# sdatkinson/NeuralAmpModelerCore

Measured on AMD Instinct MI355X. Metric: real-time audio streams (xRT) at 48 kHz, wavenet_a1_standard, higher is better.
Workload: dtype f32

## Files before the change

neuralampmodelercore_amd/csrc/aq_table.h:

```cpp
#pragma once

namespace namhip
{
namespace aq
{
constexpr int kC0 = 16, kC1 = 8;
constexpr int kBlockF = 64;
constexpr int kLayers = 10;
constexpr int kJobT = 10, kJobM0 = 11, kJobHead = 21, kJobs = 22;
constexpr int kRings = 20;
constexpr int kTable = 64;
constexpr int kNst = 16;
constexpr int kFirst[kNst + 1] = {0, 1, 2, 3, 4, 5, 6, 7, 8, 9, 10, 12, 14, 16, 18, 20, 22};
#ifdef NAM_AQ_SOW
constexpr int kStageOfWave[kNst] = {NAM_AQ_SOW};
#else
constexpr int kStageOfWave[kNst] = {0, 3, 6, 8, 1, 4, 7, 9, 2, 5, 11, 13, 15, 10, 12, 14};
#endif
static_assert(kFirst[kNst] == kJobs, "aq stage table");

constexpr bool is_big(int job) { return job < kLayers; }
constexpr bool is_small(int job) { return job >= kJobM0 && job < kJobHead; }
constexpr bool has_ring(int job) { return is_big(job) || is_small(job); }
constexpr int ring_id(int job) { return is_big(job) ? job : job - kJobM0 + kLayers; }
constexpr int dil(int job) { return has_ring(job) ? 1 << (is_big(job) ? job : job - kJobM0) : 0; }
constexpr int chans(int job) { return job <= kJobT ? kC0 : kC1; }
constexpr int ring_len(int job) { return 2 * dil(job) + kBlockF; }
constexpr int ring_off(int job)
{
  int o = kTable;
  for (int r = 0; r < ring_id(job); r++)
    o += (r < kLayers ? kC0 : kC1) * (2 * (1 << (r % kLayers)) + kBlockF);
  return o;
}
constexpr bool res(int job) { return is_big(job) ? dil(job) <= 64 : is_small(job) ? dil(job) <= 128 : false; }
constexpr int stage_of(int job)
{
  int s = 0;
  for (int k = 1; k < kNst; k++)
    if (job >= kFirst[k])
      s = k;
  return s;
}
constexpr bool starts_stage(int job) { return kFirst[stage_of(job)] == job; }
constexpr bool takes_area(int job) { return job > 0 && job < kJobHead && starts_stage(job) && !res(job); }
#if defined(NAM_AQ_DEPTH4_MASK)
constexpr int depth_in(int job) { return (is_big(job) && ((NAM_AQ_DEPTH4_MASK >> job) & 1)) ? 4 : 2; }
#elif defined(NAM_AQ_DEEP_Q)
constexpr int depth_in(int job) { return (is_big(job) && !res(job)) ? 4 : 2; }
#else
constexpr int depth_in(int) { return 2; }
#endif
constexpr int kMirror = 15;
constexpr int mirror_rows(int job) { return is_big(job) && res(job) ? kMirror : 0; }
constexpr int in_rows(int job) { return res(job) ? ring_len(job) + mirror_rows(job) : takes_area(job) ? (is_big(job) ? 16 * depth_in(job) : kBlockF) : 0; }
constexpr int plane_b(int job) { return (in_rows(job) * 16 + 255) / 256 * 256; }
constexpr int in_bytes(int job) { return plane_b(job) * (chans(job) / 4); }

constexpr int kTileT = 4 * 2 * 16;
constexpr int kTileM = 4 * 2 * 8;
constexpr int kWrOff = 0;
constexpr int kWhOff = kWrOff + kTileT;
constexpr int kMTiles = kWhOff + kTileT;
constexpr int kHeadTile = kMTiles + kLayers * 4 * kTileM;
constexpr int kMConsts = kHeadTile + kTileM;
constexpr int kTConsts = kMConsts + kLayers * 24;
constexpr int kBigConsts = kTConsts + 16;
constexpr int kBlockFloats = kBigConsts + kLayers * 64;
static_assert(kBlockFloats % 4 == 0, "aq weight block");

constexpr int kWB = 0;
constexpr int kFlagB = kWB + kBlockFloats * 4;
constexpr int kSlotB0 = kFlagB + 256;
constexpr int kSubSlot = 2 * 1024 + 128 + 16, kBigSlot = 4 * 1024 + 256 + 16, kSmallSlot = 2 * 1024 + 256 + 16;
constexpr int slot_bytes(int b) { return is_big(kFirst[b + 1]) ? (depth_in(kFirst[b + 1]) == 4 ? kBigSlot : kSubSlot) : kFirst[b + 1] == kJobT ? kBigSlot : kSmallSlot; }
constexpr int slot_b(int b)
{
  int o = kSlotB0;
  for (int i = 0; i < b; i++)
    o += slot_bytes(i);
  return o;
}
constexpr int kInB0 = (slot_b(kNst - 1) + 255) / 256 * 256;
constexpr int in_b(int job)
{
  int o = kInB0;
  for (int i = 0; i < job; i++)
    o += in_bytes(i);
  return o;
}
constexpr int kLdsBytes = in_b(kJobs);
static_assert(kLdsBytes <= 160 * 1024, "aq LDS layout");
constexpr bool mirrors_fit()
{
  for (int j = 0; j < kJobs; j++)
    if (mirror_rows(j) && ((ring_len(j) + kMirror) * 16 > plane_b(j) || ring_len(j) < 2 * 16 + kMirror))
      return false;
  return true;
}
static_assert(mirrors_fit(), "aq: a mirror lies behind its ring's live rows, inside the ring's plane");
static_assert(kFlagB % 16 == 0 && kSlotB0 % 16 == 0 && kSubSlot % 16 == 0 && kBigSlot % 16 == 0 && kSmallSlot % 16 == 0, "aq LDS alignment");
}
}
```

neuralampmodelercore_amd/csrc/kernel_a1_q.hip:

```cpp
#include "device_common.h"
#include "il_common.h"
#include "aq_table.h"

#ifndef NAM_AQ_SLEEP
#define NAM_AQ_SLEEP 1
#endif
#define NAM_AQ_STR2(x) #x
#define NAM_AQ_STR(x) NAM_AQ_STR2(x)

namespace namhip
{

constexpr float kAqT1 = 0.893229853513558f, kAqT2 = (float)(2.45550750702956 - 2.44506634652299 * 0.893229853513558);
#pragma clang fp contract(off)
template <int ACT_T>
__device__ __forceinline__ mf::f4 aq_act4(const mf::f4& v, float c_t1 = kAqT1, float c_t2 = kAqT2)
{
  mf::f4 r;
#pragma unroll
  for (int i = 0; i < 4; i++)
  {
    const float x = v[i];
    if constexpr (ACT_T == ACT_FASTTANH)
    {
      constexpr float kA1 = (float)(2.45550750702956 - 2.44506634652299 * 0.821226666969744);
      const float ax = __builtin_fabsf(x);
      const float q = __builtin_fmaf(ax, ax, 2.44506634652299f);
      const float w = __builtin_fmaf(0.814642734961073f, ax, 1.0f);
      const float t1 = __builtin_fmaf(0.821226666969744f, ax, c_t1);
      const float t2 = __builtin_fmaf(kA1, ax, c_t2);
      const float den = __builtin_fmaf(q, ax * w, 2.44506634652299f);
      const float n = __builtin_fmaf(t1, q, t2);
      r[i] = (n * __builtin_amdgcn_rcpf(den)) * x;
    }
    else
    {
      static_assert(ACT_T == ACT_TANH, "nam_a1_q_kernel is compiled for Fasttanh and Tanh");
      const float e = __builtin_amdgcn_exp2f(x * 2.885390081777927f);
      r[i] = __builtin_fmaf(-2.0f, __builtin_amdgcn_rcpf(e + 1.0f), 1.0f);
    }
  }
  return r;
}

#ifdef NAM_AQ_STEADY_PRIO
constexpr int kAqSteadyPrio[aq::kNst] = {NAM_AQ_STEADY_PRIO};
#else
constexpr int kAqSteadyPrio[aq::kNst] = {0, 0, 0, 0, 0, 0, 0, 0, 0, 0, 0, 0, 0, 0, 0, 0};
#endif
template <int SS>
__device__ __forceinline__ void aq_steady_prio()
{
  if constexpr (kAqSteadyPrio[SS] == 3)
    __builtin_amdgcn_s_setprio((short)3);
  else if constexpr (kAqSteadyPrio[SS] == 2)
    __builtin_amdgcn_s_setprio((short)2);
  else if constexpr (kAqSteadyPrio[SS] == 1)
    __builtin_amdgcn_s_setprio((short)1);
  else
    __builtin_amdgcn_s_setprio((short)0);
}

#ifndef NAM_AQ_STAG_SLEEP
#define NAM_AQ_STAG_SLEEP 24
#endif
template <int SS>
__device__ __forceinline__ void aq_stagger()
{
#ifdef NAM_AQ_STAG_FIXED
  if constexpr (SS > 0)
    __builtin_amdgcn_s_sleep(NAM_AQ_STAG_FIXED);
#endif
  if constexpr (SS > 0 && NAM_AQ_STAG_SLEEP > 0)
  {
#pragma unroll 1
    for (int r = 0; r < SS; r++)
      __builtin_amdgcn_s_sleep(NAM_AQ_STAG_SLEEP);
  }
}

namespace aq
{
constexpr int kNotReady = -(1 << 20);
constexpr int kNoRow = 1 << 26;
constexpr int kRowsMax = 1 << 20;
constexpr int far_jobs_before(int s, int job)
{
  int c = 0;
  for (int i = kFirst[s]; i < job; i++)
    c += (has_ring(i) && !res(i)) ? 1 : 0;
  return c;
}
constexpr int max_far_small()
{
  int m = 0;
  for (int s = 0; s < kNst; s++)
    if (is_small(kFirst[s]))
      m = far_jobs_before(s, kFirst[s + 1]) > m ? far_jobs_before(s, kFirst[s + 1]) : m;
  return m;
}
}

template <int ACT_T, bool WT, bool PERSIST, bool DBG = false, bool BANK = false>
__global__ __launch_bounds__(aq::kNst * 64) void nam_a1_q_kernel(const float* __restrict__ blob0, const A1Args a)
{
  long long dbg_t[8] = {0, 0, 0, 0, 0, 0, 0, 0};
  if constexpr (DBG)
    dbg_t[0] = clock64();
  using namespace mf;
  using il::kOob;
  using il::i4;
  constexpr int NST = aq::kNst;
  extern __shared__ __attribute__((aligned(16))) float lds_aq[];
  char* const lds = reinterpret_cast<char*>(lds_aq);
  const int tid = threadIdx.x;
  const int lane = tid & 63;
  const int wall = uni(tid >> 6);
  int S = 0;
#pragma unroll
  for (int i = 0; i < NST; i++)
    S = wall == i ? aq::kStageOfWave[i] : S;
  __builtin_amdgcn_s_setprio((short)0);
  if (wall >= 12)
    __builtin_amdgcn_s_setprio((short)3);
  else if (wall >= 8)
    __builtin_amdgcn_s_setprio((short)2);
  else if (wall >= 4)
    __builtin_amdgcn_s_setprio((short)1);
  const int stream = a.stream_map ? a.stream_map[blockIdx.x] : (int)blockIdx.x;
  const il::Weights wsrc = il::weights_of<BANK>(blob0, a, stream);
  const float* __restrict__ blob = wsrc.blob;
  float* st = a.state + (size_t)stream * a.state_stride;
  const int n_blocks = PERSIST ? (1 << 30) : (a.n_frames + kBlock - 1) / kBlock;

  const int frame = lane;
  const int g = lane >> 4, n = lane & 15;
  const unsigned g16 = (unsigned)g * 16u;
  const unsigned frame16 = (unsigned)frame * 16u;
  const unsigned cls64 = (unsigned)(lane & 3) * 64u;
  const unsigned cls128 = (unsigned)(lane & 3) * 128u;
  const float* in = a.in ? a.in + (size_t)stream * a.io_stride : nullptr;
  float* out = a.out ? a.out + (size_t)stream * a.io_stride : nullptr;
  const float head_scale = wsrc.head_scale;
  const int io_bytes = PERSIST ? 0x7ffffff0 : a.n_frames * 4;
  const auto rsrc_in = __builtin_amdgcn_make_buffer_rsrc((void*)(in ? in : st), 0, in ? io_bytes : 0, 0x00020000);
  const auto rsrc_out = __builtin_amdgcn_make_buffer_rsrc((void*)(out ? out : st), 0, out ? io_bytes : 0, 0x00020000);
  const unsigned long long in_addr = (unsigned long long)(in ? in : st);
  const i4 in_desc = {uni((int)(unsigned)in_addr), uni((int)(unsigned)(in_addr >> 32) & 0xffff), in ? io_bytes : 0, 0x00020000};
  int* wpos_tbl = reinterpret_cast<int*>(st);
  const int wposv = lane < aq::kRings ? wpos_tbl[lane] : 0;
  int* const flags = reinterpret_cast<int*>(lds + aq::kFlagB);

  constexpr int NT = 64;
  auto copy_block = [&](int first_float, int n_floats) {
    const f4* __restrict__ src = reinterpret_cast<const f4*>(blob + a.tiles_off + first_float);
    const int n4 = n_floats / 4;
    for (int i0 = 0; i0 < n4; i0 += 2 * NT)
    {
      const f4 t0 = src[min(i0 + lane, n4 - 1)], t1 = src[min(i0 + NT + lane, n4 - 1)];
      if (i0 + lane < n4)
        lds_st4(lds, (unsigned)aq::kWB + (unsigned)(first_float * 4) + (unsigned)(i0 + lane) * 16u, t0);
      if (i0 + NT + lane < n4)
        lds_st4(lds, (unsigned)aq::kWB + (unsigned)(first_float * 4) + (unsigned)(i0 + NT + lane) * 16u, t1);
    }
  };

  const i4 rs16 = il::ring_desc(st, aq::kC0 * 4, aq::kRowsMax), rs8 = il::ring_desc(st, aq::kC1 * 4, aq::kRowsMax);
  using il::wrap_row;
  using il::wrap_s;

  constexpr bool kOutHost = PERSIST && WT;
  constexpr int kInAux = PERSIST ? 17 : 0;
#ifdef NAM_AQ_NO_WT
  constexpr int kAppAux = WT && !PERSIST ? 17 : 0;
  constexpr int kWbAux = 0;
#else
  constexpr int kAppAux = (WT || PERSIST) ? 17 : 0;
  constexpr int kWbAux = PERSIST ? 17 : 0;
#endif
  auto ring_load = [&](unsigned s_) {
    return __hip_atomic_load(a.p_ring + (s_ & (unsigned)a.p_ring_mask), __ATOMIC_RELAXED, __HIP_MEMORY_SCOPE_SYSTEM);
  };
  const unsigned flag_b = (unsigned)aq::kFlagB;
  auto wait_word = [&](unsigned byte_addr, int want) {
    int tmp, stmp;
    want = uni(want);
    asm volatile("1:\n\tds_read_b32 %0, %2\n\ts_waitcnt lgkmcnt(0)\n\tv_readfirstlane_b32 %1, %0\n\ts_sub_i32 %1, %1, %3\n\t"
                 "s_cmp_lt_i32 %1, 0\n\ts_cbranch_scc0 2f\n\ts_sleep " NAM_AQ_STR(NAM_AQ_SLEEP) "\n\ts_branch 1b\n2:"
                 : "=&v"(tmp), "=&s"(stmp)
                 : "v"(byte_addr), "s"(want)
                 : "scc");
  };
  auto wait_in = [&](unsigned byte_addr, int want) {
    if constexpr (DBG)
    {
      const long long t0 = clock64();
      wait_word(byte_addr, want);
      dbg_t[5] += clock64() - t0;
    }
    else
      wait_word(byte_addr, want);
  };
  auto wait_out = [&](unsigned byte_addr, int want) {
    if constexpr (DBG)
    {
      const long long t0 = clock64();
      wait_word(byte_addr, want);
      dbg_t[6] += clock64() - t0;
    }
    else
      wait_word(byte_addr, want);
  };
  auto set_word = [&](unsigned byte_addr, int v) {
    asm volatile("" ::: "memory");
    if (lane == 0)
      __hip_atomic_store(reinterpret_cast<int*>(lds + byte_addr), v, __ATOMIC_RELAXED, __HIP_MEMORY_SCOPE_WORKGROUP);
    asm volatile("" ::: "memory");
  };
  auto prod_b = [&](int b) { return flag_b + (unsigned)(16 + 2 * b) * 4u; };
  auto cons_b = [&](int b) { return flag_b + (unsigned)(16 + 2 * b + 1) * 4u; };

  using lds_f4_ptr = __attribute__((address_space(3))) mf::f4*;
  using lds_f_ptr = __attribute__((address_space(3))) float*;
  const unsigned lds0 = (unsigned)(size_t)(__attribute__((address_space(3))) char*)lds_aq;
  auto lds_ld4_at = [](unsigned addr) { return *(lds_f4_ptr)(size_t)addr; };
  auto lds_st4_at = [](unsigned addr, const mf::f4& v) { *(lds_f4_ptr)(size_t)addr = v; };
  auto sreg = [](unsigned v) {
    asm("" : "+s"(v));
    return v;
  };
  auto store_rows = [&](auto r_tag, unsigned lane_b, int so, const mf::f4& v) {
    constexpr int R = decltype(r_tag)::value;
    const unsigned at = lane_b + sreg((unsigned)so * 16u);
    lds_st4_at(at, v);
    if (so < aq::kMirror || so > R - 16)
    {
      const bool low = so < aq::kMirror;
      const int thr = (low ? aq::kMirror : R) - so;
      const int d = (lane & 15) < thr ? (low ? R * 16 : 0) : (low ? 0 : -R * 16);
      lds_st4_at(at + (unsigned)d, v);
    }
  };
  auto far_load = [&](i4 rs, auto r_tag, int t, int voff, int ring_off_b, int row_b) {
    constexpr int R = decltype(r_tag)::value;
    mf::f4 v;
    if (t + 16 <= R)
      v = il::sb_load4(rs, lane & 15, voff, ring_off_b + t * row_b, 0);
    else
    {
      v = il::sb_load4(rs, (int)wrap_row(t, (unsigned)(lane & 15), R), voff, ring_off_b, 0);
      asm volatile("" ::: "memory");
    }
    return v;
  };

  auto ring_to_lds = [&](auto r_tag, int ring_off_f, unsigned lds_b, unsigned plane_b, auto wide_tag) {
    constexpr int R = decltype(r_tag)::value;
    constexpr bool wide = decltype(wide_tag)::value;
    constexpr int per = wide ? 16 : 32, NI = (R + per - 1) / per;
    const int rl = wide ? n : (lane >> 1);
    const unsigned pl = wide ? (unsigned)g : (unsigned)(lane & 1);
    f4 t[NI];
#pragma unroll
    for (int i = 0; i < NI; i++)
    {
      const int row = i * per + rl;
      t[i] = il::sb_load4(wide ? rs16 : rs8, row < R ? row : aq::kNoRow, (int)(pl * 16u), ring_off_f * 4, 0);
    }
#pragma unroll
    for (int i = 0; i < NI; i++)
    {
      const int row = i * per + rl;
      if (row < R)
        lds_st4(lds, lds_b + pl * plane_b + (unsigned)row * 16u, t[i]);
      if (wide && i == 0 && row < aq::kMirror)
        lds_st4(lds, lds_b + pl * plane_b + (unsigned)(R + row) * 16u, t[i]);
    }
  };
  auto lds_to_ring = [&](auto r_tag, int ring_off_f, unsigned lds_b, unsigned plane_b, auto wide_tag) {
    constexpr int R = decltype(r_tag)::value;
    constexpr bool wide = decltype(wide_tag)::value;
    constexpr int per = wide ? 16 : 32, NI = (R + per - 1) / per;
    const int rl = wide ? n : (lane >> 1);
    const unsigned pl = wide ? (unsigned)g : (unsigned)(lane & 1);
    f4 t[NI];
#pragma unroll
    for (int i = 0; i < NI; i++)
      t[i] = lds_ld4(lds, lds_b + pl * plane_b + (unsigned)min(i * per + rl, R - 1) * 16u);
#pragma unroll
    for (int i = 0; i < NI; i++)
    {
      const int row = i * per + rl;
      il::sb_store4(t[i], wide ? rs16 : rs8, row < R ? row : aq::kNoRow, (int)(pl * 16u), ring_off_f * 4, kWbAux);
    }
  };

  unsigned na = 0;
  unsigned done = 0;
  unsigned boff0 = 0;
  if (tid < 64)
    flags[tid] = (tid >= 17 && tid < 17 + 2 * (NST - 1) && (tid & 1)) ? aq::kNotReady : 0;
  lds_barrier();
  if constexpr (PERSIST)
  {
    const bool by_value = a.p_seq0 >= 0;
    done = na = by_value ? (unsigned)a.p_seq0 : a.p_cons[blockIdx.x];
    bool ready = true;
    unsigned lo = (unsigned)a.p_cmd0;
    if (!by_value)
    {
      if (wall == 0)
      {
        unsigned long long v = session_wait_command<8>(a, ring_load, na + 1u, ring_load(na), (long long)a.p_grace);
        if (lane == 0)
        {
          flags[48] = (int)(unsigned)v;
          flags[49] = (unsigned)(v >> 32) == na + 1 ? 1 : 0;
        }
      }
      lds_barrier();
      ready = uni(flags[49]) != 0;
      lo = (unsigned)uni(flags[48]);
      lds_barrier();
    }
    if (!ready)
    {
      if (wall == 0 && lane == 0)
      {
        session_leaving(a);
        a.p_cons[blockIdx.x] = done;
        __hip_atomic_store(a.p_done + blockIdx.x, done | 0x80000000u, __ATOMIC_RELAXED, __HIP_MEMORY_SCOPE_SYSTEM);
      }
      return;
    }
    boff0 = lo * 4u;
  }

  int nvalid = kBlock;
  bool more = false;
  unsigned boff = 0;
  auto store_positions = [&](int r0, int nr, const int* wpv) {
    int v = 0;
#pragma unroll
    for (int u = 0; u < 5; u++)
      v = (u < nr && lane == r0 + u) ? wpv[u < nr ? u : 0] : v;
    if (lane >= r0 && lane < r0 + nr)
      wpos_tbl[lane] = v;
  };

  auto run_big = [&](auto s_tag) {
    constexpr int SS = decltype(s_tag)::value;
    constexpr int J0 = aq::kFirst[SS], NJS = aq::kFirst[SS + 1] - J0, JN = aq::kFirst[SS + 1];
    constexpr bool FIRST = SS == 0;
    constexpr int QIN = SS - 1, QOUT = SS;
    constexpr int NFAR = aq::far_jobs_before(SS, JN);
    constexpr int DIN = aq::depth_in(J0), DOUT = JN == aq::kJobT ? 4 : aq::depth_in(JN);
    static_assert(aq::is_big(JN) || JN == aq::kJobT, "aq: array 0's last stage hands over to the transition");
    aq_stagger<SS>();
    f4 W[NJS][4];
    {
      const f4* __restrict__ tsrc = reinterpret_cast<const f4*>(blob + a.consts_off);
#pragma unroll
      for (int u = 0; u < NJS; u++)
#pragma unroll
        for (int q = 0; q < 4; q++)
          W[u][q] = tsrc[(J0 + u) * 256 + q * 64 + lane];
    }
    int wp[NJS];
#pragma unroll
    for (int u = 0; u < NJS; u++)
      wp[u] = __builtin_amdgcn_readlane(wposv, aq::ring_id(J0 + u));
    int wpo = aq::res(JN) ? __builtin_amdgcn_readlane(wposv, aq::ring_id(aq::res(JN) ? JN : 0)) : 0;
    unsigned gb[NJS];
#pragma unroll
    for (int u = 0; u < NJS; u++)
      gb[u] = (unsigned)aq::in_b(J0 + u) + (unsigned)g * (unsigned)aq::plane_b(J0 + u);
    const unsigned gbn = (unsigned)aq::in_b(JN) + (unsigned)g * (unsigned)aq::plane_b(JN);
    const unsigned n16 = lds0 + (unsigned)n * 16u;
    unsigned gl[NJS];
#pragma unroll
    for (int u = 0; u < NJS; u++)
      gl[u] = gb[u] + n16;
    const unsigned gln = gbn + n16;
    constexpr unsigned islot_ = (unsigned)aq::slot_b(QIN < 0 ? 0 : QIN), oslot_ = (unsigned)aq::slot_b(QOUT);
    const unsigned hd_in = islot_ + g16 * (unsigned)(DIN * 16) + n16, cnd_in = lds0 + islot_ + (unsigned)(DIN * 1024) + (unsigned)n * 4u;
    const unsigned hd_out = oslot_ + g16 * (unsigned)(DOUT * 16) + n16, cnd_out = lds0 + oslot_ + (unsigned)(DOUT * 1024) + (unsigned)n * 4u;
    il::for_each_index(
      [&](auto u_tag) {
        constexpr int TJ = J0 + decltype(u_tag)::value;
        if constexpr (aq::res(TJ))
          ring_to_lds(std::integral_constant<int, aq::ring_len(TJ)>{}, aq::ring_off(TJ), (unsigned)aq::in_b(TJ), (unsigned)aq::plane_b(TJ), std::true_type{});
      },
      std::make_integer_sequence<int, NJS>{});
    f4 far[NFAR > 0 ? NFAR : 1][2];
    auto fetch_far = [&](auto tj_tag, int sb) {
      constexpr int TJ = decltype(tj_tag)::value;
      constexpr int R = aq::ring_len(TJ), D = aq::dil(TJ), FI = aq::far_jobs_before(SS, TJ);
#pragma unroll
      for (int j = 0; j < 2; j++)
        far[FI][j] = far_load(rs16, std::integral_constant<int, R>{}, wrap_s(sb - (2 - j) * D, R), (int)g16, aq::ring_off(TJ) * 4, aq::kC0 * 4);
    };
    il::for_each_index(
      [&](auto u_tag) {
        constexpr int TJ = J0 + decltype(u_tag)::value;
        if constexpr (!aq::res(TJ))
          fetch_far(std::integral_constant<int, TJ>{}, wp[TJ - J0]);
      },
      std::make_integer_sequence<int, NJS>{});
    float inp = 0.0f;
    if constexpr (FIRST)
      inp = __builtin_bit_cast(float, __builtin_amdgcn_raw_buffer_load_b32(rsrc_in, frame * 4, uni((int)boff0), kInAux));
    f4 cst[NJS][3];
    f4 rech = {0.f, 0.f, 0.f, 0.f};
    {
      const f4* __restrict__ csrc = reinterpret_cast<const f4*>(blob + a.tiles_off + aq::kBigConsts);
#pragma unroll
      for (int u = 0; u < NJS; u++)
#pragma unroll
        for (int q = 0; q < 3; q++)
          cst[u][q] = csrc[(J0 + u) * 16 + q * 4 + g];
      if constexpr (FIRST)
        rech = csrc[12 + g];
    }
    __builtin_amdgcn_s_waitcnt(0);
    if constexpr (!FIRST)
      set_word(cons_b(QIN), 0);
    if constexpr (DBG)
      dbg_t[1] = clock64();

    float c_t1 = kAqT1, c_t2 = kAqT2;
    asm volatile("" : "+v"(c_t1), "+v"(c_t2));
    f4 xs, hd;
    float cnd = 0.0f;
    unsigned long long spec_cmd = 0;
    float inp_spec = 0.0f;
    int k = 0;
    int m = 0;
    int i = 0;
    int m1 = 0;

    auto job = [&](auto j_tag) {
      constexpr int JI = decltype(j_tag)::value;
      constexpr int U = JI - J0;
      constexpr int R = aq::ring_len(JI), D = aq::dil(JI);
      constexpr bool RES = aq::res(JI);
      constexpr bool TAKES = U == 0 && SS > 0;
      constexpr int FI = aq::far_jobs_before(SS, JI);
      __builtin_amdgcn_sched_barrier(0);
      const int wpj = wp[U];
      int sb = wpj + 16 * i;
      sb -= sb >= R ? R : 0;
      if constexpr (TAKES)
        xs = lds_ld4_at(gl[U] + sreg(RES ? (unsigned)sb * 16u : (unsigned)(m & (DIN - 1)) * 256u));
      else if constexpr (RES)
      {
        store_rows(std::integral_constant<int, R>{}, gl[U], sb, xs);
        asm volatile("" ::: "memory");
      }
      if constexpr (!RES)
      {
        if ((PERSIST || 16 * i + 16 <= nvalid) && sb + 16 <= R)
          il::sb_store4(xs, rs16, n, (int)g16, aq::ring_off(JI) * 4 + sb * (aq::kC0 * 4), kAppAux);
        else
        {
          il::sb_store4(xs, rs16, (PERSIST || 16 * i + n < nvalid) ? (int)wrap_row(sb, (unsigned)n, R) : aq::kNoRow, (int)g16, aq::ring_off(JI) * 4, kAppAux);
          asm volatile("" ::: "memory");
        }
      }
      f4 bt[2];
#pragma unroll
      for (int j = 0; j < 2; j++)
      {
        if constexpr (RES)
          bt[j] = lds_ld4_at(gl[U] + sreg((unsigned)wrap_s(sb - (2 - j) * D, R) * 16u));
        else
          bt[j] = far[FI][j];
      }
      if constexpr (TAKES)
        set_word(cons_b(QIN), m1);
      if constexpr (PERSIST && JI == 0)
      {
        if (i == 0)
        {
          const unsigned long long v = ring_load(na + 1);
          spec_cmd = ((unsigned long long)(unsigned)uni((int)(unsigned)(v >> 32)) << 32) | (unsigned long long)(unsigned)uni((int)(unsigned)v);
        }
        if (i == 2)
        {
          const bool hit = (unsigned)(spec_cmd >> 32) == na + 2;
          const int soff = uni(hit ? (int)((unsigned)spec_cmd * 4u) : 0);
          inp_spec = __builtin_bit_cast(float, __builtin_amdgcn_raw_buffer_load_b32(rsrc_in, hit ? frame * 4 : (int)kOob, soff, kInAux));
        }
      }
      const f4 bv = cst[U][0], mv = cst[U][1];
      f4 acc = __builtin_elementwise_fma(mv, f4{cnd, cnd, cnd, cnd}, bv);
#pragma unroll
      for (int s_ = 0; s_ < 4; s_++)
        acc = __builtin_amdgcn_mfma_f32_16x16x4f32(W[U][0][s_], bt[0][s_], acc, 0, 0, 0);
#pragma unroll
      for (int s_ = 0; s_ < 4; s_++)
        acc = __builtin_amdgcn_mfma_f32_16x16x4f32(W[U][1][s_], bt[1][s_], acc, 0, 0, 0);
      if constexpr (!RES)
      {
        int wpn_ = wpj + nvalid;
        wpn_ -= wpn_ >= R ? R : 0;
        int nsb = sb + 16;
        nsb -= nsb >= R ? R : 0;
        fetch_far(j_tag, i == 3 ? wpn_ : nsb);
      }
#pragma unroll
      for (int s_ = 0; s_ < 4; s_++)
        acc = __builtin_amdgcn_mfma_f32_16x16x4f32(W[U][2][s_], xs[s_], acc, 0, 0, 0);
      const f4 b1v = cst[U][2];
      const f4 z = aq_act4<ACT_T>(acc, c_t1, c_t2);
      hd += z;
      xs += b1v;
#pragma unroll
      for (int s_ = 0; s_ < 4; s_++)
        xs = __builtin_amdgcn_mfma_f32_16x16x4f32(W[U][3][s_], z[s_], xs, 0, 0, 0);
    };

    boff = boff0;
    bool have = !FIRST || n_blocks > 0;
#pragma unroll 1
    for (;; k++)
    {
      bool exit_tok = false;
      float cond = 0.0f;
      constexpr unsigned islot = (unsigned)aq::slot_b(QIN < 0 ? 0 : QIN), oslot = (unsigned)aq::slot_b(QOUT);
      if constexpr (FIRST)
      {
        exit_tok = !have;
        nvalid = PERSIST ? kBlock : min(kBlock, a.n_frames - k * kBlock);
        more = PERSIST || k + 1 < n_blocks;
      }
      else
      {
        wait_in(prod_b(QIN), m + 1);
        asm volatile("" ::: "memory");
        const i4 tok = *reinterpret_cast<const i4*>(lds + islot + (unsigned)(DIN * 1024 + DIN * 64));
        boff = (unsigned)uni(tok[0]);
        nvalid = uni(tok[1]);
        exit_tok = uni(tok[2]) != 0;
        more = PERSIST || uni(tok[3]) != 0;
      }
      if (exit_tok)
      {
        wait_out(cons_b(QOUT), m - (DOUT - 1));
        asm volatile("" ::: "memory");
        if (lane == 0)
          *reinterpret_cast<i4*>(lds + oslot + (unsigned)(DOUT * 1024 + DOUT * 64)) = i4{(int)boff, nvalid, 1, 0};
        set_word(prod_b(QOUT), m + 1);
        break;
      }
      if constexpr (FIRST)
      {
        cond = inp;
        if constexpr (!PERSIST)
          inp = __builtin_bit_cast(float, __builtin_amdgcn_raw_buffer_load_b32(rsrc_in, frame * 4, uni((k + 1) * (kBlock * 4)), 0));
      }
#pragma unroll 1
      for (i = 0; i < 4; i++)
      {
        unsigned a_hd = 0, a_cnd = 0;
        asm volatile("v_mov_b32 %0, %1" : "=v"(m1) : "s"(m + 1));
        if constexpr (FIRST)
        {
          cnd = __builtin_bit_cast(float, __builtin_amdgcn_ds_bpermute((16 * i + n) * 4, __builtin_bit_cast(int, cond)));
          xs = rech * cnd;
          hd = f4{0.f, 0.f, 0.f, 0.f};
        }
        else
        {
          if (i > 0)
          {
            wait_in(prod_b(QIN), m + 1);
            asm volatile("" ::: "memory");
          }
          const unsigned qs = (unsigned)(m & (DIN - 1));
          a_hd = hd_in + sreg(qs * 256u);
          a_cnd = cnd_in + sreg(qs * 64u);
          hd = lds_ld4_at(a_hd);
          cnd = *(lds_f_ptr)(size_t)a_cnd;
        }
        il::for_each_index([&](auto u_tag) { job(std::integral_constant<int, J0 + decltype(u_tag)::value>{}); },
                           std::make_integer_sequence<int, NJS>{});
        wait_out(cons_b(QOUT), m - (DOUT - 1));
        asm volatile("" ::: "memory");
        {
          int so = wpo + 16 * i;
          so -= (aq::res(JN) && so >= aq::ring_len(JN)) ? aq::ring_len(JN) : 0;
          const unsigned qs = (unsigned)(m & (DOUT - 1));
          if constexpr (aq::res(JN))
            store_rows(std::integral_constant<int, aq::ring_len(JN)>{}, gln, so, xs);
          else
            lds_st4_at(gln + sreg(qs * 256u), xs);
          if constexpr (FIRST || DIN != DOUT)
          {
            a_hd = hd_out + sreg(qs * 256u) - (oslot_ - islot_);
            a_cnd = cnd_out + sreg(qs * 64u) - (oslot_ - islot_);
          }
          lds_st4_at(a_hd + (oslot_ - islot_), hd);
          if (g == 0)
            *(lds_f_ptr)(size_t)(a_cnd + (oslot_ - islot_)) = cnd;
          if (i == 0)
          {
            asm volatile("" ::: "memory");
            if (lane == 0)
              *reinterpret_cast<i4*>(lds + oslot + (unsigned)(DOUT * 1024 + DOUT * 64)) = i4{(int)boff, nvalid, 0, more ? 1 : 0};
          }
        }
        set_word(prod_b(QOUT), m1);
        m = (int)((unsigned)m + 1u);
        if constexpr (DBG)
        {
          dbg_t[3] = clock64();
          dbg_t[2] = dbg_t[2] ? dbg_t[2] : dbg_t[3];
          dbg_t[7] = m;
        }
      }
      if (k == 0)
        aq_steady_prio<SS>();
#pragma unroll
      for (int u = 0; u < NJS; u++)
      {
        int np = wp[u] + nvalid;
        np -= np >= aq::ring_len(J0 + u) ? aq::ring_len(J0 + u) : 0;
        wp[u] = np;
      }
      if constexpr (aq::res(JN))
      {
        wpo += nvalid;
        wpo -= wpo >= aq::ring_len(JN) ? aq::ring_len(JN) : 0;
      }
      if constexpr (FIRST)
      {
        if constexpr (PERSIST)
        {
          const unsigned tag = na + 2u;
          unsigned long long v = spec_cmd;
          if ((unsigned)(v >> 32) != tag)
          {
            v = session_wait_command<16>(a, ring_load, tag, ring_load(tag - 1u), (long long)(a.p_linger > 0 ? a.p_linger : 100));
          }
          const unsigned v_tag = (unsigned)uni((int)(unsigned)(v >> 32)), v_off = (unsigned)uni((int)(unsigned)v);
          have = v_tag == tag;
          if (!have && lane == 0)
            session_leaving(a);
          const unsigned next_off = v_off * 4u;
          na++;
          if (have)
          {
            boff = next_off;
            const bool mine = (unsigned)(spec_cmd >> 32) == na + 1u && (unsigned)spec_cmd * 4u == next_off;
            inp = inp_spec;
            if (!mine)
            {
              const int voff = frame * 4, soff = uni((int)next_off);
              const i4 rsd = in_desc;
              asm volatile("buffer_load_dword %0, %1, %2, %3 offen sc0 sc1\n\ts_waitcnt vmcnt(0)"
                           : "=v"(inp)
                           : "v"(voff), "s"(rsd), "s"(soff)
                           : "memory");
            }
          }
        }
        else
        {
          have = k + 1 < n_blocks;
          boff = (unsigned)(k + 1) * (kBlock * 4u);
        }
      }
    }
    asm volatile("" ::: "memory");
    il::for_each_index(
      [&](auto u_tag) {
        constexpr int TJ = J0 + decltype(u_tag)::value;
        if constexpr (aq::res(TJ))
          lds_to_ring(std::integral_constant<int, aq::ring_len(TJ)>{}, aq::ring_off(TJ), (unsigned)aq::in_b(TJ), (unsigned)aq::plane_b(TJ), std::true_type{});
      },
      std::make_integer_sequence<int, NJS>{});
    store_positions(aq::ring_id(J0), NJS, wp);
  };

  auto run_small = [&](auto s_tag) {
    constexpr int SS = decltype(s_tag)::value;
    constexpr int J0 = aq::kFirst[SS], JE = aq::kFirst[SS + 1];
    constexpr bool LAST = SS == NST - 1, HAS_T = J0 == aq::kJobT;
    constexpr int JM0 = HAS_T ? J0 + 1 : J0;
    constexpr int NL = (LAST ? JE - 1 : JE) - JM0;
    constexpr int JN = LAST ? JM0 : JE;
    constexpr int QIN = SS - 1, QOUT = SS;
    constexpr int NFAR = aq::far_jobs_before(SS, JM0 + NL);
    static_assert(NL >= 1 && (LAST || aq::is_small(JN)), "aq: small stages hold layers");
    aq_stagger<SS>();
    int wp[NL];
#pragma unroll
    for (int u = 0; u < NL; u++)
      wp[u] = __builtin_amdgcn_readlane(wposv, aq::ring_id(JM0 + u));
    int wpo = (!LAST && aq::res(JN)) ? __builtin_amdgcn_readlane(wposv, aq::ring_id(JN)) : 0;
    il::for_each_index(
      [&](auto u_tag) {
        constexpr int TJ = JM0 + decltype(u_tag)::value;
        if constexpr (aq::res(TJ))
          ring_to_lds(std::integral_constant<int, aq::ring_len(TJ)>{}, aq::ring_off(TJ), (unsigned)aq::in_b(TJ), (unsigned)aq::plane_b(TJ), std::false_type{});
      },
      std::make_integer_sequence<int, NL>{});
    struct Row
    {
      f4 q0, q1;
    };
    Row far[NFAR > 0 ? NFAR : 1][2];
    auto fetch_far = [&](auto tj_tag, int wpj) {
      constexpr int TJ = decltype(tj_tag)::value;
      constexpr int R = aq::ring_len(TJ), D = aq::dil(TJ), FI = aq::far_jobs_before(SS, TJ);
#pragma unroll
      for (int j = 0; j < 2; j++)
      {
        const int idx = (int)wrap_row(wrap_s(wpj - (2 - j) * D, R), (unsigned)frame, R);
        far[FI][j].q0 = il::sb_load4(rs8, idx, 0, aq::ring_off(TJ) * 4, 0);
        far[FI][j].q1 = il::sb_load4(rs8, idx, 16, aq::ring_off(TJ) * 4, 0);
      }
    };
    il::for_each_index(
      [&](auto u_tag) {
        constexpr int TJ = JM0 + decltype(u_tag)::value;
        if constexpr (!aq::res(TJ))
          fetch_far(std::integral_constant<int, TJ>{}, wp[TJ - JM0]);
      },
      std::make_integer_sequence<int, NL>{});
    copy_block(aq::kMTiles + (JM0 - aq::kJobM0) * 4 * aq::kTileM, NL * 4 * aq::kTileM);
    copy_block(aq::kMConsts + (JM0 - aq::kJobM0) * 24, NL * 24);
    if constexpr (HAS_T)
      copy_block(aq::kWrOff, 2 * aq::kTileT);
    if constexpr (LAST)
      copy_block(aq::kHeadTile, aq::kTileM);
    if constexpr (HAS_T || LAST)
      copy_block(aq::kTConsts, 16);
    __builtin_amdgcn_s_waitcnt(0);
    set_word(cons_b(QIN), 0);
    if constexpr (DBG)
      dbg_t[1] = clock64();

    f4 x0, x1, head0, head1;
    float cond = 0.0f;
    int k = 0;
    auto job = [&](auto j_tag) {
      constexpr int JI = decltype(j_tag)::value;
      constexpr int U = JI - JM0, LI = JI - aq::kJobM0;
      constexpr int R = aq::ring_len(JI), D = aq::dil(JI);
      constexpr bool RES = aq::res(JI), TAKES = U == 0 && !HAS_T;
      constexpr int FI = aq::far_jobs_before(SS, JI);
      constexpr unsigned rb0 = (unsigned)aq::in_b(JI), rb1 = rb0 + (unsigned)aq::plane_b(JI);
      __builtin_amdgcn_sched_barrier(0);
      const int wpj = wp[U];
      const unsigned row0 = wrap_row(wpj, (unsigned)frame, R);
      if constexpr (TAKES)
      {
        const unsigned r_in = RES ? row0 * 16u : frame16;
        x0 = lds_ld4(lds, rb0 + r_in);
        x1 = lds_ld4(lds, rb1 + r_in);
      }
      else if constexpr (RES)
      {
        lds_st4(lds, rb0 + row0 * 16u, x0);
        lds_st4(lds, rb1 + row0 * 16u, x1);
        asm volatile("" ::: "memory");
      }
      if constexpr (!RES)
      {
        const int widx = frame < nvalid ? (int)row0 : aq::kNoRow;
        il::sb_store4(x0, rs8, widx, 0, aq::ring_off(JI) * 4, kAppAux);
        il::sb_store4(x1, rs8, widx, 16, aq::ring_off(JI) * 4, kAppAux);
      }
      int wpn = wpj + nvalid;
      wpn -= wpn >= R ? R : 0;
      f4 b0[2], b1[2];
#pragma unroll
      for (int j = 0; j < 2; j++)
      {
        if constexpr (RES)
        {
          const unsigned row = wrap_row(wrap_s(wpj - (2 - j) * D, R), (unsigned)frame, R) * 16u;
          b0[j] = lds_ld4(lds, rb0 + row);
          b1[j] = lds_ld4(lds, rb1 + row);
        }
        else
          b0[j] = far[FI][j].q0, b1[j] = far[FI][j].q1;
      }
      if constexpr (TAKES)
        set_word(cons_b(QIN), k + 1);
      constexpr unsigned cb = (unsigned)(aq::kWB + (aq::kMConsts + LI * 24) * 4);
      f4 acc0 = lds_ld4(lds, cb), acc1 = lds_ld4(lds, cb + 16u);
      {
        const f4 m0 = lds_ld4(lds, cb + 32u), m1 = lds_ld4(lds, cb + 48u);
        const f4 c4 = {cond, cond, cond, cond};
        acc0 = __builtin_elementwise_fma(m0, c4, acc0);
        acc1 = __builtin_elementwise_fma(m1, c4, acc1);
      }
      struct Tile
      {
        f4 a, b, c, d;
      };
      auto tile_ld = [&](unsigned tb) { return Tile{lds_ld4(lds, tb + cls64), lds_ld4(lds, tb + 16u + cls64), lds_ld4(lds, tb + 32u + cls64), lds_ld4(lds, tb + 48u + cls64)}; };
      auto tap = [&](const Tile& w, const f4& v0, const f4& v1, f4& o0, f4& o1) {
#pragma unroll
        for (int c = 0; c < 4; c++)
        {
          o0 = __builtin_amdgcn_mfma_f32_4x4x1f32(w.a[c], v0[c], o0, 0, 0, 0);
          o1 = __builtin_amdgcn_mfma_f32_4x4x1f32(w.c[c], v0[c], o1, 0, 0, 0);
        }
#pragma unroll
        for (int c = 0; c < 4; c++)
        {
          o0 = __builtin_amdgcn_mfma_f32_4x4x1f32(w.b[c], v1[c], o0, 0, 0, 0);
          o1 = __builtin_amdgcn_mfma_f32_4x4x1f32(w.d[c], v1[c], o1, 0, 0, 0);
        }
      };
      constexpr unsigned t0 = (unsigned)(aq::kWB + (aq::kMTiles + LI * 4 * aq::kTileM) * 4);
      const Tile w0 = tile_ld(t0), w1 = tile_ld(t0 + 256u);
      tap(w0, b0[0], b1[0], acc0, acc1);
      const Tile w2 = tile_ld(t0 + 512u);
      tap(w1, b0[1], b1[1], acc0, acc1);
      if constexpr (!RES)
        fetch_far(j_tag, wpn);
      const Tile w3 = tile_ld(t0 + 768u);
      tap(w2, x0, x1, acc0, acc1);
      const f4 b1v0 = lds_ld4(lds, cb + 64u), b1v1 = lds_ld4(lds, cb + 80u);
      const f4 z0 = aq_act4<ACT_T>(acc0), z1 = aq_act4<ACT_T>(acc1);
      head0 += z0;
      head1 += z1;
      f4 y0 = x0 + b1v0, y1 = x1 + b1v1;
      tap(w3, z0, z1, y0, y1);
      x0 = y0;
      x1 = y1;
      wp[U] = wpn;
    };

#pragma unroll 1
    for (;; k++)
    {
      constexpr unsigned slot = (unsigned)aq::slot_b(QIN), oslot = (unsigned)aq::slot_b(LAST ? QIN : QOUT);
      i4 tok;
      bool exit_tok;
      if constexpr (HAS_T)
      {
        constexpr unsigned xin = (unsigned)aq::in_b(aq::kJobT);
        const int m0 = (int)(4u * (unsigned)k);
        wait_in(prod_b(QIN), m0 + 1);
        asm volatile("" ::: "memory");
        tok = *reinterpret_cast<const i4*>(lds + slot + 4352u);
        exit_tok = uni(tok[2]) != 0;
        if (!exit_tok)
          wait_in(prod_b(QIN), m0 + 4);
        asm volatile("" ::: "memory");
        f4 x16[4], h16[4];
#pragma unroll
        for (int p = 0; p < 4; p++)
        {
          x16[p] = lds_ld4(lds, xin + (unsigned)p * 1024u + frame16);
          h16[p] = lds_ld4(lds, slot + (unsigned)p * 1024u + frame16);
        }
        cond = *reinterpret_cast<const float*>(lds + slot + 4096u + (unsigned)lane * 4u);
        set_word(cons_b(QIN), m0 + 4);
        constexpr unsigned wr = (unsigned)(aq::kWB + aq::kWrOff * 4), wh = (unsigned)(aq::kWB + aq::kWhOff * 4), tc = (unsigned)(aq::kWB + aq::kTConsts * 4);
        x0 = x1 = f4{0.f, 0.f, 0.f, 0.f};
        head0 = lds_ld4(lds, tc);
        head1 = lds_ld4(lds, tc + 16u);
#pragma unroll
        for (int p = 0; p < 4; p++)
        {
          const f4 w0 = lds_ld4(lds, wr + cls128 + (unsigned)p * 16u), w1 = lds_ld4(lds, wr + cls128 + 64u + (unsigned)p * 16u);
#pragma unroll
          for (int c = 0; c < 4; c++)
          {
            x0 = __builtin_amdgcn_mfma_f32_4x4x1f32(w0[c], x16[p][c], x0, 0, 0, 0);
            x1 = __builtin_amdgcn_mfma_f32_4x4x1f32(w1[c], x16[p][c], x1, 0, 0, 0);
          }
        }
#pragma unroll
        for (int p = 0; p < 4; p++)
        {
          const f4 w0 = lds_ld4(lds, wh + cls128 + (unsigned)p * 16u), w1 = lds_ld4(lds, wh + cls128 + 64u + (unsigned)p * 16u);
#pragma unroll
          for (int c = 0; c < 4; c++)
          {
            head0 = __builtin_amdgcn_mfma_f32_4x4x1f32(w0[c], h16[p][c], head0, 0, 0, 0);
            head1 = __builtin_amdgcn_mfma_f32_4x4x1f32(w1[c], h16[p][c], head1, 0, 0, 0);
          }
        }
      }
      else
      {
        wait_in(prod_b(QIN), k + 1);
        asm volatile("" ::: "memory");
        tok = *reinterpret_cast<const i4*>(lds + slot + 2304u);
        head0 = lds_ld4(lds, slot + frame16);
        head1 = lds_ld4(lds, slot + 1024u + frame16);
        cond = *reinterpret_cast<const float*>(lds + slot + 2048u + (unsigned)lane * 4u);
        exit_tok = uni(tok[2]) != 0;
      }
      boff = (unsigned)uni(tok[0]);
      nvalid = uni(tok[1]);
      if (exit_tok)
      {
        if constexpr (!HAS_T)
          set_word(cons_b(QIN), k + 1);
        if constexpr (!LAST)
        {
          wait_out(cons_b(QOUT), k);
          asm volatile("" ::: "memory");
          if (lane == 0)
            *reinterpret_cast<i4*>(lds + oslot + 2304u) = tok;
          set_word(prod_b(QOUT), k + 1);
        }
        break;
      }
      il::for_each_index([&](auto u_tag) { job(std::integral_constant<int, JM0 + decltype(u_tag)::value>{}); },
                         std::make_integer_sequence<int, NL>{});
      if constexpr (DBG)
      {
        dbg_t[3] = clock64();
        dbg_t[2] = dbg_t[2] ? dbg_t[2] : dbg_t[3];
        dbg_t[7] = k + 1;
      }
      if (k == 0)
        aq_steady_prio<SS>();
      if constexpr (!LAST)
      {
        constexpr int RN = aq::ring_len(JN);
        wait_out(cons_b(QOUT), k);
        asm volatile("" ::: "memory");
        const unsigned row = aq::res(JN) ? wrap_row(wpo, (unsigned)frame, RN) * 16u : frame16;
        lds_st4(lds, (unsigned)aq::in_b(JN) + row, x0);
        lds_st4(lds, (unsigned)(aq::in_b(JN) + aq::plane_b(JN)) + row, x1);
        lds_st4(lds, oslot + frame16, head0);
        lds_st4(lds, oslot + 1024u + frame16, head1);
        *reinterpret_cast<float*>(lds + oslot + 2048u + (unsigned)lane * 4u) = cond;
        if (lane == 0)
          *reinterpret_cast<i4*>(lds + oslot + 2304u) = tok;
        if constexpr (aq::res(JN))
        {
          wpo += nvalid;
          wpo -= wpo >= RN ? RN : 0;
        }
        set_word(prod_b(QOUT), k + 1);
      }
      else
      {
        constexpr unsigned tb = (unsigned)(aq::kWB + aq::kHeadTile * 4);
        const f4 wa = lds_ld4(lds, tb + cls64), wb = lds_ld4(lds, tb + 16u + cls64);
        f4 acc = lds_ld4(lds, (unsigned)(aq::kWB + aq::kTConsts * 4) + 32u);
#pragma unroll
        for (int c = 0; c < 4; c++)
          acc = __builtin_amdgcn_mfma_f32_4x4x1f32(wa[c], head0[c], acc, 0, 0, 0);
#pragma unroll
        for (int c = 0; c < 4; c++)
          acc = __builtin_amdgcn_mfma_f32_4x4x1f32(wb[c], head1[c], acc, 0, 0, 0);
        const float yout = head_scale * acc[0];
        if (kOutHost && a.p_out_host == 2)
          __builtin_amdgcn_raw_buffer_store_b32(__builtin_bit_cast(unsigned, yout), rsrc_out, frame < nvalid ? frame * 4 : (int)kOob, uni((int)boff), 17);
        else
          __builtin_amdgcn_raw_buffer_store_b32(__builtin_bit_cast(unsigned, yout), rsrc_out, frame < nvalid ? frame * 4 : (int)kOob, uni((int)boff),
                                                PERSIST && !kOutHost ? 17 : 0);
        if constexpr (PERSIST)
        {
          done++;
          if (kOutHost && a.p_out_host == 2)
          {
            asm volatile("s_waitcnt vmcnt(0)" ::: "memory");
            unsigned before = 0u;
            const unsigned cslot = (done - 1u) & (unsigned)a.p_ring_mask;
            if (lane == 0)
              before = __hip_atomic_fetch_add(a.p_cmd_count + cslot, 1u, __ATOMIC_RELAXED, __HIP_MEMORY_SCOPE_AGENT);
            if ((unsigned)uni((int)before) == gridDim.x - 1u && lane == 0)
            {
              __hip_atomic_store(a.p_cmd_count + cslot, 0u, __ATOMIC_RELAXED, __HIP_MEMORY_SCOPE_AGENT);
              __hip_atomic_store(a.p_cmd_done + cslot, done, __ATOMIC_RELAXED, __HIP_MEMORY_SCOPE_SYSTEM);
              __hip_atomic_fetch_max(a.p_cmd_count + a.p_ring_mask + 1, done, __ATOMIC_RELAXED, __HIP_MEMORY_SCOPE_AGENT);
            }
            if (lane == 0 && (done & 15u) == 0u)
              __hip_atomic_store(a.p_prog + blockIdx.x, done, __ATOMIC_RELAXED, __HIP_MEMORY_SCOPE_SYSTEM);
          }
          else if (lane == 0 && (done & 15u) == 0u)
            __hip_atomic_store(a.p_prog + blockIdx.x, done, __ATOMIC_RELAXED, __HIP_MEMORY_SCOPE_SYSTEM);
        }
      }
    }
    asm volatile("" ::: "memory");
    il::for_each_index(
      [&](auto u_tag) {
        constexpr int TJ = JM0 + decltype(u_tag)::value;
        if constexpr (aq::res(TJ))
          lds_to_ring(std::integral_constant<int, aq::ring_len(TJ)>{}, aq::ring_off(TJ), (unsigned)aq::in_b(TJ), (unsigned)aq::plane_b(TJ), std::false_type{});
      },
      std::make_integer_sequence<int, NL>{});
    store_positions(aq::ring_id(JM0), NL, wp);
  };

  il::for_each_index(
    [&](auto s_tag) {
      constexpr int SS = decltype(s_tag)::value;
      if (S == SS)
      {
        if constexpr (aq::is_big(aq::kFirst[SS]))
          run_big(s_tag);
        else
          run_small(s_tag);
      }
    },
    std::make_integer_sequence<int, NST>{});

  if constexpr (DBG)
  {
    dbg_t[4] = clock64();
    if (a.dbg && blockIdx.x == 0 && lane < 8)
    {
      long long v = 0;
#pragma unroll
      for (int i = 0; i < 8; i++)
        v = lane == i ? dbg_t[i] : v;
      a.dbg[S * 8 + lane] = v;
    }
  }
  if constexpr (PERSIST)
  {
    asm volatile("s_waitcnt vmcnt(0)" ::: "memory");
    lds_barrier();
    if constexpr (kOutHost)
    {
      if (S == NST - 1)
        __builtin_amdgcn_fence(__ATOMIC_RELEASE, "");
    }
    if (S == NST - 1 && lane == 0)
    {
      a.p_cons[blockIdx.x] = done;
      __hip_atomic_store(a.p_done + blockIdx.x, done | 0x80000000u, __ATOMIC_RELAXED, __HIP_MEMORY_SCOPE_SYSTEM);
    }
  }
}

#ifdef NAM_AQ_PROBE
template __global__ void nam_a1_q_kernel<ACT_FASTTANH, false, true>(const float* __restrict__, const A1Args);
#else
namespace
{
template <int ACT_T, bool BANK>
hipError_t launch_q_bank(const A1Args& a, int n_blocks, LaunchStream stream)
{
  return with_session_form(a.p_ring != nullptr, a.p_out_host != 0, a.n_frames, [&](auto wt, auto persist) {
    return launch_instance<&nam_a1_q_kernel<ACT_T, decltype(wt)::value, decltype(persist)::value, false, BANK>>(
      dim3(n_blocks), dim3(aq::kNst * 64), aq::kLdsBytes, stream, a.blob, a);
  });
}
}

bool a1_q_takes(int act)
{
  return act == ACT_FASTTANH || act == ACT_TANH;
}
hipError_t launch_a1_q(const A1Args& a, int n_blocks, int act, LaunchStream stream)
{
  if (a.dbg && !a.p_ring && !a.bank_member)
    return launch_instance<&nam_a1_q_kernel<ACT_FASTTANH, false, false, true>>(dim3(n_blocks), dim3(aq::kNst * 64), aq::kLdsBytes, stream.stream, a.blob, a);
  const bool bank = a.bank_member != nullptr;
  if (act == ACT_FASTTANH)
    return bank ? launch_q_bank<ACT_FASTTANH, true>(a, n_blocks, stream) : launch_q_bank<ACT_FASTTANH, false>(a, n_blocks, stream);
  if (act == ACT_TANH)
    return bank ? launch_q_bank<ACT_TANH, true>(a, n_blocks, stream) : launch_q_bank<ACT_TANH, false>(a, n_blocks, stream);
  return hipErrorInvalidValue;
}
#endif

}
```

Measured before the change: 64950.

## Step ring byte offsets incrementally, prefetch queue flags, drop lane-0 guards

```diff
diff --git a/neuralampmodelercore_amd/csrc/aq_table.h b/neuralampmodelercore_amd/csrc/aq_table.h
--- a/neuralampmodelercore_amd/csrc/aq_table.h
+++ b/neuralampmodelercore_amd/csrc/aq_table.h
@@ -53,6 +53,19 @@
 #endif
 constexpr int kMirror = 15;
 constexpr int mirror_rows(int job) { return is_big(job) && res(job) ? kMirror : 0; }
+constexpr unsigned kSubB = 16u * 16u;
+constexpr unsigned ring_b(int job) { return (unsigned)ring_len(job) * 16u; }
+constexpr unsigned pos_b(int pos, int back, int R)
+{
+  const int v = pos - back;
+  return (unsigned)(v < 0 ? v + R : v) * 16u;
+}
+constexpr unsigned step_b(unsigned off, unsigned rb)
+{
+  const unsigned a = off + kSubB, b = a - rb;
+  return a < b ? a : b;
+}
+constexpr bool mirror_b(unsigned off, unsigned rb) { return off < (unsigned)kMirror * 16u || off > rb - kSubB; }
 constexpr int in_rows(int job) { return res(job) ? ring_len(job) + mirror_rows(job) : takes_area(job) ? (is_big(job) ? 16 * depth_in(job) : kBlockF) : 0; }
 constexpr int plane_b(int job) { return (in_rows(job) * 16 + 255) / 256 * 256; }
 constexpr int in_bytes(int job) { return plane_b(job) * (chans(job) / 4); }
diff --git a/neuralampmodelercore_amd/csrc/kernel_a1_q.hip b/neuralampmodelercore_amd/csrc/kernel_a1_q.hip
--- a/neuralampmodelercore_amd/csrc/kernel_a1_q.hip
+++ b/neuralampmodelercore_amd/csrc/kernel_a1_q.hip
@@ -5,6 +5,7 @@
 #ifndef NAM_AQ_SLEEP
 #define NAM_AQ_SLEEP 1
 #endif
+constexpr bool kAqMathFence = true;
 #define NAM_AQ_STR2(x) #x
 #define NAM_AQ_STR(x) NAM_AQ_STR2(x)
 
@@ -211,10 +212,19 @@
     else
       wait_word(byte_addr, want);
   };
+  auto look_word = [&](unsigned byte_addr) {
+    asm volatile("" ::: "memory");
+    const int v = __hip_atomic_load(reinterpret_cast<const int*>(lds + byte_addr), __ATOMIC_RELAXED, __HIP_MEMORY_SCOPE_WORKGROUP);
+    asm volatile("" ::: "memory");
+    return v;
+  };
+  auto wait_looked = [&](int seen, unsigned byte_addr, int want) {
+    if ((int)((unsigned)uni(seen) - (unsigned)uni(want)) < 0)
+      wait_in(byte_addr, want);
+  };
   auto set_word = [&](unsigned byte_addr, int v) {
     asm volatile("" ::: "memory");
-    if (lane == 0)
-      __hip_atomic_store(reinterpret_cast<int*>(lds + byte_addr), v, __ATOMIC_RELAXED, __HIP_MEMORY_SCOPE_WORKGROUP);
+    __hip_atomic_store(reinterpret_cast<int*>(lds + byte_addr), v, __ATOMIC_RELAXED, __HIP_MEMORY_SCOPE_WORKGROUP);
     asm volatile("" ::: "memory");
   };
   auto prod_b = [&](int b) { return flag_b + (unsigned)(16 + 2 * b) * 4u; };
@@ -229,12 +239,13 @@
     asm("" : "+s"(v));
     return v;
   };
-  auto store_rows = [&](auto r_tag, unsigned lane_b, int so, const mf::f4& v) {
+  auto store_rows = [&](auto r_tag, unsigned lane_b, unsigned so_b, const mf::f4& v) {
     constexpr int R = decltype(r_tag)::value;
-    const unsigned at = lane_b + sreg((unsigned)so * 16u);
+    const unsigned at = lane_b + sreg(so_b);
     lds_st4_at(at, v);
-    if (so < aq::kMirror || so > R - 16)
-    {
+    if (aq::mirror_b(so_b, (unsigned)R * 16u))
+    {
+      const int so = (int)(so_b >> 4);
       const bool low = so < aq::kMirror;
       const int thr = (low ? aq::kMirror : R) - so;
       const int d = (lane & 15) < thr ? (low ? R * 16 : 0) : (low ? 0 : -R * 16);
@@ -371,6 +382,16 @@
     for (int u = 0; u < NJS; u++)
       wp[u] = __builtin_amdgcn_readlane(wposv, aq::ring_id(J0 + u));
     int wpo = aq::res(JN) ? __builtin_amdgcn_readlane(wposv, aq::ring_id(aq::res(JN) ? JN : 0)) : 0;
+    unsigned ob[NJS][3], ob_out = 0;
+    auto offsets_from_positions = [&]() {
+#pragma unroll
+      for (int u = 0; u < NJS; u++)
+#pragma unroll
+        for (int q = 0; q < 3; q++)
+          ob[u][q] = aq::pos_b(wp[u], q == 0 ? 0 : (3 - q) * aq::dil(J0 + u), aq::ring_len(J0 + u));
+      ob_out = (unsigned)wpo * 16u;
+    };
+    offsets_from_positions();
     unsigned gb[NJS];
 #pragma unroll
     for (int u = 0; u < NJS; u++)
@@ -438,6 +459,12 @@
     int m = 0;
     int i = 0;
     int m1 = 0;
+    int seen_in = 0;
+    auto sub_block = [&]() {
+      int v = i;
+      asm volatile("" : "+s"(v));
+      return v;
+    };
 
     auto job = [&](auto j_tag) {
       constexpr int JI = decltype(j_tag)::value;
@@ -447,14 +474,20 @@
       constexpr bool TAKES = U == 0 && SS > 0;
       constexpr int FI = aq::far_jobs_before(SS, JI);
       __builtin_amdgcn_sched_barrier(0);
+      constexpr bool STEPS = RES;
       const int wpj = wp[U];
-      int sb = wpj + 16 * i;
-      sb -= sb >= R ? R : 0;
+      int sb = 0;
+      if constexpr (!STEPS)
+      {
+        sb = wpj + 16 * i;
+        sb -= sb >= R ? R : 0;
+      }
+      const unsigned sb_b = STEPS ? ob[U][0] : (unsigned)sb * 16u;
       if constexpr (TAKES)
-        xs = lds_ld4_at(gl[U] + sreg(RES ? (unsigned)sb * 16u : (unsigned)(m & (DIN - 1)) * 256u));
+        xs = lds_ld4_at(gl[U] + sreg(RES ? sb_b : (unsigned)(m & (DIN - 1)) * 256u));
       else if constexpr (RES)
       {
-        store_rows(std::integral_constant<int, R>{}, gl[U], sb, xs);
+        store_rows(std::integral_constant<int, R>{}, gl[U], sb_b, xs);
         asm volatile("" ::: "memory");
       }
       if constexpr (!RES)
@@ -471,10 +504,18 @@
 #pragma unroll
       for (int j = 0; j < 2; j++)
       {
-        if constexpr (RES)
+        if constexpr (STEPS)
+          bt[j] = lds_ld4_at(gl[U] + sreg(ob[U][1 + j]));
+        else if constexpr (RES)
           bt[j] = lds_ld4_at(gl[U] + sreg((unsigned)wrap_s(sb - (2 - j) * D, R) * 16u));
         else
           bt[j] = far[FI][j];
+      }
+      if constexpr (STEPS)
+      {
+#pragma unroll
+        for (int q = 0; q < 3; q++)
+          ob[U][q] = aq::step_b(ob[U][q], aq::ring_b(JI));
       }
       if constexpr (TAKES)
         set_word(cons_b(QIN), m1);
@@ -512,6 +553,10 @@
       for (int s_ = 0; s_ < 4; s_++)
         acc = __builtin_amdgcn_mfma_f32_16x16x4f32(W[U][2][s_], xs[s_], acc, 0, 0, 0);
       const f4 b1v = cst[U][2];
+      if constexpr (kAqMathFence && RES && SS > 0)
+        asm volatile("" : "+v"(xs), "+v"(acc));
+      else if constexpr (kAqMathFence && JN == aq::kJobT)
+        asm volatile("" : "+v"(xs));
       const f4 z = aq_act4<ACT_T>(acc, c_t1, c_t2);
       hd += z;
       xs += b1v;
@@ -536,7 +581,7 @@
       }
       else
       {
-        wait_in(prod_b(QIN), m + 1);
+        wait_looked(seen_in, prod_b(QIN), m + 1);
         asm volatile("" ::: "memory");
         const i4 tok = *reinterpret_cast<const i4*>(lds + islot + (unsigned)(DIN * 1024 + DIN * 64));
         boff = (unsigned)uni(tok[0]);
@@ -548,8 +593,7 @@
       {
         wait_out(cons_b(QOUT), m - (DOUT - 1));
         asm volatile("" ::: "memory");
-        if (lane == 0)
-          *reinterpret_cast<i4*>(lds + oslot + (unsigned)(DOUT * 1024 + DOUT * 64)) = i4{(int)boff, nvalid, 1, 0};
+        *reinterpret_cast<i4*>(lds + oslot + (unsigned)(DOUT * 1024 + DOUT * 64)) = i4{(int)boff, nvalid, 1, 0};
         set_word(prod_b(QOUT), m + 1);
         break;
       }
@@ -572,9 +616,9 @@
         }
         else
         {
-          if (i > 0)
+          if (sub_block() > 0)
           {
-            wait_in(prod_b(QIN), m + 1);
+            wait_looked(seen_in, prod_b(QIN), m + 1);
             asm volatile("" ::: "memory");
           }
           const unsigned qs = (unsigned)(m & (DIN - 1));
@@ -587,12 +631,21 @@
                            std::make_integer_sequence<int, NJS>{});
         wait_out(cons_b(QOUT), m - (DOUT - 1));
         asm volatile("" ::: "memory");
-        {
-          int so = wpo + 16 * i;
-          so -= (aq::res(JN) && so >= aq::ring_len(JN)) ? aq::ring_len(JN) : 0;
+        if constexpr (!FIRST)
+          seen_in = look_word(prod_b(QIN));
+        {
+          unsigned so_b = ob_out;
+          if constexpr (aq::res(JN))
+            ob_out = aq::step_b(ob_out, aq::ring_b(JN));
+          else
+          {
+            int so = wpo + 16 * i;
+            so -= (aq::res(JN) && so >= aq::ring_len(JN)) ? aq::ring_len(JN) : 0;
+            so_b = (unsigned)so * 16u;
+          }
           const unsigned qs = (unsigned)(m & (DOUT - 1));
           if constexpr (aq::res(JN))
-            store_rows(std::integral_constant<int, aq::ring_len(JN)>{}, gln, so, xs);
+            store_rows(std::integral_constant<int, aq::ring_len(JN)>{}, gln, so_b, xs);
           else
             lds_st4_at(gln + sreg(qs * 256u), xs);
           if constexpr (FIRST || DIN != DOUT)
@@ -603,11 +656,10 @@
           lds_st4_at(a_hd + (oslot_ - islot_), hd);
           if (g == 0)
             *(lds_f_ptr)(size_t)(a_cnd + (oslot_ - islot_)) = cnd;
-          if (i == 0)
+          if (sub_block() == 0)
           {
             asm volatile("" ::: "memory");
-            if (lane == 0)
-              *reinterpret_cast<i4*>(lds + oslot + (unsigned)(DOUT * 1024 + DOUT * 64)) = i4{(int)boff, nvalid, 0, more ? 1 : 0};
+            *reinterpret_cast<i4*>(lds + oslot + (unsigned)(DOUT * 1024 + DOUT * 64)) = i4{(int)boff, nvalid, 0, more ? 1 : 0};
           }
         }
         set_word(prod_b(QOUT), m1);
@@ -632,6 +684,11 @@
       {
         wpo += nvalid;
         wpo -= wpo >= aq::ring_len(JN) ? aq::ring_len(JN) : 0;
+      }
+      if constexpr (!PERSIST)
+      {
+        if (nvalid != kBlock)
+          offsets_from_positions();
       }
       if constexpr (FIRST)
       {
@@ -910,8 +967,7 @@
         {
           wait_out(cons_b(QOUT), k);
           asm volatile("" ::: "memory");
-          if (lane == 0)
-            *reinterpret_cast<i4*>(lds + oslot + 2304u) = tok;
+          *reinterpret_cast<i4*>(lds + oslot + 2304u) = tok;
           set_word(prod_b(QOUT), k + 1);
         }
         break;
@@ -937,8 +993,7 @@
         lds_st4(lds, oslot + frame16, head0);
         lds_st4(lds, oslot + 1024u + frame16, head1);
         *reinterpret_cast<float*>(lds + oslot + 2048u + (unsigned)lane * 4u) = cond;
-        if (lane == 0)
-          *reinterpret_cast<i4*>(lds + oslot + 2304u) = tok;
+        *reinterpret_cast<i4*>(lds + oslot + 2304u) = tok;
         if constexpr (aq::res(JN))
         {
           wpo += nvalid;
```

After: 64620 (median of 2 runs). Within noise of the previous version (-0.5%).
